# jolars/sgdnet

Measured on AMD Instinct MI355X. Metric: saga_epochs_per_sec, higher is better.
Workload: dtype f64

## Files before the change

sgdnet_amd/csrc/saga_batched.hip:

```cpp
#include <hip/hip_ext.h>
#include <stdlib.h>

#include <mutex>
#include <set>
#include <type_traits>
#include <utility>

#include "device_math.hpp"
#include "r_rng_word.hpp"
#include "r_rng_bodies.hpp"

#ifndef SGDNET_BIN_BLOCK
#define SGDNET_BIN_BLOCK 1024
#endif
#ifndef SGDNET_BIN_W
#define SGDNET_BIN_W 8
#endif
#ifndef SGDNET_RANGE_BLOCK
#define SGDNET_RANGE_BLOCK 512
#endif

namespace sgdnet {

namespace {
// ... 423 lines not shown
    }
    if (y_in_tag && y[i] != 0.0) bits |= 2u;
    if (bits) atomicOr(meta + (i >> 4), bits << (2 * (i & 15)));
  }
}

__global__ __launch_bounds__(256) void m_move_kernel(SagaDev d, int to_record) {
  for (int64_t i = (int64_t)blockIdx.x * 256 + threadIdx.x; i < d.n; i += (int64_t)gridDim.x * 256) {
    double* r = reinterpret_cast<double*>(d.cP + (size_t)i * kCStride + kCMOff);
    if (to_record) *r = d.M[i];
    else d.M[i] = *r;
  }
}

template <class F>
__device__ __forceinline__ void row_tail_compact(const SagaDev& d, uint32_t sid, int nnz, int gl, int E, F f) {
  const char* qb = d.cQ + (size_t)sid * kCStride;
  for (int e = E + 4 + gl; e < nnz; e += kLanes8) {
    if (e < E + kCQ) {
      f((int64_t) reinterpret_cast<const uint16_t*>(qb + 8)[e - E],
        reinterpret_cast<const double*>(qb + 32)[e - E]);
    } else {
      const int64_t q0 = d.ptr[sid];
      f((int64_t)d.idx[q0 + e], d.val[q0 + e]);
    }
  }
}

#ifndef SGDNET_LDS_BLOCK
#define SGDNET_LDS_BLOCK 1024
#endif
constexpr int kLdsBlock = SGDNET_LDS_BLOCK;

constexpr int kTicket = 32;

struct TicketSource {
  int* counter;
  int lo, hi, m;
  int t = 0;
  bool dynamic;
  __device__ __forceinline__ int next() {
    if (!dynamic) {
      const int b = lo + (t++ * (kLdsBlock / 64) + (int)(threadIdx.x >> 6)) * kTicket;
      return b < hi ? b : m;
    }
    int b = 0;
    if ((threadIdx.x & 63) == 0)
      b = __hip_atomic_fetch_add(counter, kTicket, __ATOMIC_RELAXED, __HIP_MEMORY_SCOPE_WORKGROUP);
    b = lo + __builtin_amdgcn_readfirstlane(b);
    return b < hi ? b : m;
  }
};

struct K1Compact {
  typedef double dpair_t __attribute__((ext_vector_type(2)));
  static constexpr int U = 4;
  int E, in_reg, gl, g, q, slot, id_off, v_off;
  bool y_in_meta, is_owner, in_p, half;
  const char* plane;
  char* P;
  const uint32_t* sp;
  const uint32_t* meta;
  int m;
  TicketSource tk;
  int b_cur, b_nxt;
  uint32_t s_cur, s_nxt;

  __device__ __forceinline__ int own_pos(int base) const { return base + U * g + q < m ? base + U * g + q : base; }
  __device__ __forceinline__ uint32_t tagged(uint32_t sid) const {
    const uint32_t mb = (meta[sid >> 4] >> (2 * (sid & 15))) & 3u;
    return sid | ((mb & 1u) ? kLongBit : 0u) | ((mb & 2u) ? kYBit : 0u);
  }
  static __device__ __forceinline__ int static_tickets() { return 2 * (kLdsBlock / 64) * kTicket; }

  __device__ __forceinline__ void init(const SagaDev& d, const uint32_t* sp_, int m_, int blk, int nblk,
                                       int* ticket_counter) {
    E = d.cE;
    in_reg = E + 4;
    y_in_meta = E == 12;
    gl = threadIdx.x & (kLanes8 - 1);
    g = (threadIdx.x & 63) >> 3;
    q = gl >> 1;
    is_owner = (gl & 1) == 0;
    in_p = gl < 6;
    slot = in_p ? gl : gl - 6;
    P = d.cP;
    plane = in_p ? d.cP : d.cQ;
    id_off = in_p ? 8 * E + 4 * slot : 8 + 4 * slot;
    v_off = in_p ? 16 * slot : 32 + 16 * slot;
    half = in_p && slot == 5 && E == 11;
    sp = sp_;
    meta = d.cmeta;
    m = m_;
    const int share = ((m + nblk - 1) / nblk + kTicket - 1) / kTicket * kTicket;
    tk.counter = ticket_counter;
    tk.lo = blk * share;
    tk.hi = tk.lo + share < m ? tk.lo + share : m;
    tk.m = m;
    tk.dynamic = share >= 4 * (kLdsBlock / 64) * kTicket;
    tk.t = 2;
    const int wave = (int)(threadIdx.x >> 6);
    b_cur = tk.lo + wave * kTicket;
    b_nxt = tk.lo + ((kLdsBlock / 64) + wave) * kTicket;
    if (b_cur >= tk.hi) b_cur = m;
    if (b_nxt >= tk.hi) b_nxt = m;
  }
  __device__ __forceinline__ void request_first() {
    s_cur = b_cur < m ? sp[own_pos(b_cur)] : 0u;
    s_nxt = b_nxt < m ? sp[own_pos(b_nxt)] : 0u;
  }
  __device__ __forceinline__ void begin(const SagaDev& d, const uint32_t* sp_, int m_, int blk, int nblk,
                                        int* ticket_counter) {
    init(d, sp_, m_, blk, nblk, ticket_counter);
    request_first();
  }

  __device__ __forceinline__ void tag_first() {
    if (b_cur < m) s_cur = tagged(s_cur);
  }

  __device__ __forceinline__ double run(const SagaDev& d, double b0, const double* wv, double* Dl) {
    double gct = 0.0;
    while (b_cur < m) {
      const bool v_own = b_cur + U * g + q < m;
      uint32_t su[U];
#pragma unroll
      for (int u = 0; u < U; ++u) su[u] = (uint32_t)__shfl((int)s_cur, 2 * u, kLanes8);
      const uint32_t s_this = s_cur & kIdMask;
      double y_own = (s_cur & kYBit) ? 1.0 : 0.0;
      if (!y_in_meta) y_own = *reinterpret_cast<const double*>(P + (size_t)s_this * kCStride + kCYOff);
      int nnz_own = 0;
      if (s_cur & kLongBit) nnz_own = *reinterpret_cast<const int*>(d.cQ + (size_t)s_this * kCStride);
      uint32_t jf[U];
      dpair_t vf[U];
#pragma unroll
      for (int u = 0; u < U; ++u) {
        const bool on = in_p || (su[u] & kLongBit) != 0;
        const char* base = plane + (size_t)(su[u] & kIdMask) * kCStride;
        jf[u] = 0u;
        vf[u] = dpair_t{0.0, 0.0};
        if (on) {
          jf[u] = *reinterpret_cast<const uint32_t*>(base + id_off);
          vf[u] = *reinterpret_cast<const dpair_t*>(base + v_off);
        }
      }
      const int b_nn = b_nxt < m ? tk.next() : m;
      uint32_t s_nn = 0u;
      if (b_nn < m) s_nn = sp[own_pos(b_nn)];
      if (b_nxt < m) s_nxt = tagged(s_nxt);
      if (half) {
#pragma unroll
        for (int u = 0; u < U; ++u) {
          vf[u].y = 0.0;
          jf[u] &= 0xffffu;
        }
      }
      double acc[U];
#pragma unroll
      for (int u = 0; u < U; ++u) acc[u] = vf[u].x * wv[jf[u] & 0xffffu] + vf[u].y * wv[jf[u] >> 16];
      const bool own_tail = v_own && nnz_own > in_reg;
      const bool any_tail = __ballot(own_tail) != 0;
      if (any_tail) {
#pragma unroll
        for (int u = 0; u < U; ++u) {
          const int nz = __shfl(own_tail ? nnz_own : 0, 2 * u, kLanes8);
          if (nz > in_reg) {
            double a = 0.0;
            row_tail_compact(d, su[u] & kIdMask, nz, gl, E, [&](int64_t j, double v) { a += v * wv[j]; });
            acc[u] += a;
          }
        }
      }
      const bool hi4 = (gl & 4) != 0, hi2 = (gl & 2) != 0;
      const double r0 = (hi4 ? acc[2] : acc[0]) + __shfl_xor(hi4 ? acc[0] : acc[2], 4, kLanes8);
      const double r1 = (hi4 ? acc[3] : acc[1]) + __shfl_xor(hi4 ? acc[1] : acc[3], 4, kLanes8);
      double t = (hi2 ? r1 : r0) + __shfl_xor(hi2 ? r0 : r1, 2, kLanes8);
      t += __shfl_xor(t, 1, kLanes8);
      const double lp = t + b0;
      const double g0 = d.family == SGDNET_BINOMIAL ? 1.0 - y_own - 1.0 / (1.0 + exp(lp)) : lp - y_own;
      double gcp = 0.0;
      if (is_owner && v_own) {
        const double old = __hip_atomic_exchange(reinterpret_cast<double*>(P + (size_t)s_this * kCStride + kCMOff), g0,
                                                 __ATOMIC_RELAXED, __HIP_MEMORY_SCOPE_AGENT);
        gcp = g0 - old;
      }
#pragma unroll
      for (int u = 0; u < U; ++u) {
        const double gc = __shfl(gcp, 2 * u, kLanes8);
        if (gc != 0.0) {
          if (vf[u].x != 0.0) scatter_add<true>(Dl + (jf[u] & 0xffffu), vf[u].x * gc);
          if (vf[u].y != 0.0) scatter_add<true>(Dl + (jf[u] >> 16), vf[u].y * gc);
          if (any_tail) {
            const int nz = __shfl(own_tail ? nnz_own : 0, 2 * u, kLanes8);
            if (nz > in_reg)
              row_tail_compact(d, su[u] & kIdMask, nz, gl, E,
                               [&](int64_t j, double v) { scatter_add<true>(Dl + j, v * gc); });
          }
        }
      }
      gct += gcp;
      s_cur = s_nxt;
      s_nxt = s_nn;
      b_cur = b_nxt;
      b_nxt = b_nn;
    }
    return gct;
  }
};

template <int U>
struct K1IdsOnly {
  uint32_t s[U];
  bool valid[U];
  uint32_t s_own;
  bool v_own;
  bool valid_any;
  __device__ __forceinline__ void load(const SagaDev& d, const uint32_t* sp, int i, int hi, int step, int gl,
                                       int safe) {
#pragma unroll
    for (int u = 0; u < U; ++u) {
      const int iu = i + u * step;
      valid[u] = iu < hi;
      s[u] = sp[valid[u] ? iu : safe];
    }
    const int q = U == 4 ? gl >> 2 : gl;
    const int iq = i + q * step;
    v_own = q < U && iq < hi;
    s_own = sp[v_own ? iq : safe];
  }
};

template <int U>
struct K1Draws {
  uint32_t s[U];
  int jf[U], nnz[U];
  double vf[U];
  double gcp;
  bool valid[U];
  uint32_t s_own;
  double y_own;
  bool v_own;
  static __device__ __forceinline__ int draw_of(int gl) { return U == 4 ? gl >> 2 : gl; }

  static __device__ __forceinline__ int owner(int u) { return U == 4 ? 4 * u : u; }
  static __device__ __forceinline__ bool is_owner(int gl) { return U == 4 ? (gl & 3) == 0 : gl < U; }

  __device__ __forceinline__ void load_ids(const SagaDev& d, const uint32_t* sp, int i, int hi, int step, int gl,
                                           int safe) {
#pragma unroll
    for (int u = 0; u < U; ++u) {
      const int iu = i + u * step;
      valid[u] = iu < hi;
      s[u] = sp[valid[u] ? iu : safe];
      if (SGD_ABLATE(d, 16)) s[u] &= 1023u;
    }
    const int q = draw_of(gl);
    const int iq = i + q * step;
    v_own = q < U && iq < hi;
    s_own = sp[v_own ? iq : safe];
    if (SGD_ABLATE(d, 16)) s_own &= 1023u;
  }
// ... 1240 lines not shown
  const int S = d.v_bps, V = d.V;
  if ((int)blockIdx.x >= V * S) {
    if (d.rngdev && lamp->rng_generate) {
      const RngDev* R = d.rngdev;
      const unsigned gen = R->gen;
      uint32_t* lds = reinterpret_cast<uint32_t*>(Dl);
      const int rb = (int)blockIdx.x - V * S, nrb = (int)gridDim.x - V * S;
      mt_state_body(rb, nrb, reinterpret_cast<uint32_t(*)[2][kMtN + 1]>(lds), R->state[gen & 1u], R->ends,
                    R->stream + (int64_t)(gen & 1u) * R->n, R->n, R->seg, R->gens);
      __syncthreads();
      mt_jump_body(rb, nrb, lds, R->state[gen & 1u], R->state[(gen + 1u) & 1u], R->poly, R->gens);
    }
    fused_leave(d, lamp, nb, false);
    return;
  }
  const int v = (int)blockIdx.x % V, wi = (int)blockIdx.x / V;
  const int F = 2 * (int)((p + 2 * S - 1) / (2 * S));
  const int j0 = wi * F;
  const int jn = p - j0 < F ? (p - j0 > 0 ? (int)(p - j0) : 0) : F;
  double* Wl = Dl + p;
  f64x2_t* D2 = reinterpret_cast<f64x2_t*>(Dl);
  f64x2_t* W2 = reinterpret_cast<f64x2_t*>(Wl);
  const int penalty = lamp->penalty;
  __shared__ double sh_par[10];
  if (tid == 0) {
    sh_par[0] = lamp->gamma;
    sh_par[1] = lamp->beta;
    sh_par[2] = lamp->r_full;
    sh_par[3] = lamp->ls_full;
    sh_par[4] = lamp->r_tail;
    sh_par[5] = lamp->ls_tail;
    double tot = 0.0, lo = 0.0;
    for (int u = 0; u < d.V; ++u) {
      tot += d.v_size[u];
      if (u < (int)blockIdx.x % d.V) lo += d.v_size[u];
    }
    sh_par[6] = d.v_size[(int)blockIdx.x % d.V];
    sh_par[7] = lo;
    sh_par[8] = tot;
  }
  const int64_t m_full = lamp->m_full;
  const int64_t sbase = lamp->stream_base;
  const bool raw_words = lamp->stream_raw != 0;
  const int64_t dps = d.v_dps;
  const bool std_x = d.standardize != 0;
  const int64_t L = 2 * p + 2;
  double* vwv = d.vw + (int64_t)v * p;
  double* vGv = d.vG + (int64_t)v * p;
  double* refv = d.vx + (int64_t)v * L;
  double* cwp = d.vx + (int64_t)V * L;
  unsigned* sync = d.vsync;
  const __amdgpu_buffer_rsrc_t rs_slab = fused_rsrc(d.slab, (int64_t)V * S * p * 8);
  const __amdgpu_buffer_rsrc_t rs_w = fused_rsrc(vwv, p * 8);
  uint32_t* const stream_v = const_cast<uint32_t*>(d.stream) + sbase + (int64_t)v * dps;
  constexpr int kC = 8;
  auto conv_range = [&](int m, int& lo, int& hi) {
    const int share = ((m + S - 1) / S + kTicket - 1) / kTicket * kTicket;
    lo = wi * share;
    hi = lo + share < m ? lo + share : m;
  };
  auto conv_load = [&](int64_t t0, int m, uint32_t (&x)[kC]) {
    int lo, hi;
    conv_range(m, lo, hi);
    const uint32_t* q = stream_v + t0;
#pragma unroll
    for (int c = 0; c < kC; ++c) {
      const int i = lo + (int)threadIdx.x + c * kLdsBlock;
      x[c] = i < hi ? q[i] : 0u;
    }
  };
  auto conv_store = [&](int64_t t0, int m, const uint32_t (&x)[kC]) {
    int lo, hi;
    conv_range(m, lo, hi);
    uint32_t* q = stream_v + t0;
    const double n_d = sh_par[6], lo_v = sh_par[7];
#pragma unroll
    for (int c = 0; c < kC; ++c) {
      const int i = lo + (int)threadIdx.x + c * kLdsBlock;
      if (i < hi) q[i] = (uint32_t)lo_v + word_to_draw(x[c], n_d);
    }
    for (int i = lo + (int)threadIdx.x + kC * kLdsBlock; i < hi; i += kLdsBlock)
      q[i] = (uint32_t)lo_v + word_to_draw(q[i], n_d);
  };

#ifdef SGDNET_PHASE_TIMING
  unsigned long long ph_t = 0;
  if (d.dbg && tid == 0) d.dbg[(size_t)blockIdx.x * 16 + 14] = ph_t = phase_stamp();
#define FPH(slot)                                                 \
  do {                                                            \
    if (d.dbg && tid == 0) {                                      \
      const unsigned long long now = phase_stamp();               \
      d.dbg[(size_t)blockIdx.x * 16 + (slot)] += now - ph_t;      \
      d.dbg[(size_t)blockIdx.x * 16 + 15] = ph_t = now;           \
    }                                                             \
  } while (0)
#else
#define FPH(slot) ((void)0)
#endif
  if (tid == 0) {
    const unsigned xcc = __builtin_amdgcn_s_getreg((3 << 11) | 20) & 15u;
    __hip_atomic_fetch_or(sync + (kSyncXcd + v) * kSyncLine, 1u << xcc, __ATOMIC_RELAXED, __HIP_MEMORY_SCOPE_AGENT);
    asm volatile("s_waitcnt vmcnt(0)" ::: "memory");
    __hip_atomic_fetch_add(sync + kSyncStart * kSyncLine, 1u, __ATOMIC_RELAXED, __HIP_MEMORY_SCOPE_AGENT);
    sh_ok = fused_start(sync, lamp, (unsigned)(V * S)) ? 1 : 0;
    if (sh_ok) {
      const unsigned mask = sync_load(sync, kSyncXcd + v);
      sh_ok = (mask & (mask - 1u)) == 0u ? 3 : 1;
    }
  }
  for (int64_t i = tid; i < P2; i += kLdsBlock) D2[i] = f64x2_t{0.0, 0.0};
  __syncthreads();
  bool done = false;
  bool alive = sh_ok != 0;
  unsigned col_base = 0u;
  if (kPeers) {
    int merges = 0;
    for (int r = 0; r < nb; ++r) merges += (r + 1 == nb || (r + 1) % every == 0) ? 1 : 0;
    col_base = sync_load(sync, kSyncSeq) * (unsigned)merges;
  }
  const bool local = (sh_ok & 2) != 0 && d.vs_xcd_local != 0;
  int mi = 0;
  uint32_t s_first = 0u, s_second = 0u;
  if (alive) {
    const int m0 = (int)(dps < m_full ? dps : m_full);
    if (raw_words) {
      uint32_t x0[kC];
      conv_load(0, m0, x0);
      conv_store(0, m0, x0);
      asm volatile("s_waitcnt vmcnt(0)" ::: "memory");
      __syncthreads();
    }
    K1Compact nx;
    nx.begin(d, stream_v, m0, wi, S, &ticket_counter);
    s_first = nx.s_cur;
    s_second = nx.s_nxt;
  }
  for (int r = 0; alive && r < nb; ++r) {
    const int64_t t0 = (int64_t)r * m_full;
    const int m = (int)(dps - t0 < m_full ? dps - t0 : m_full);
    const bool tail = m != m_full;
    const bool last = r + 1 == nb;
    const bool merge_due = last || (r + 1) % every == 0;

    if (tid == 0) ticket_counter = K1Compact::static_tickets();
    K1Compact cg;
    cg.init(d, stream_v + t0, m, wi, S, &ticket_counter);
    cg.s_cur = s_first;
    cg.s_nxt = s_second;
    cg.tag_first();
    int ts = threadIdx.x;
    asm volatile("" : "+v"(ts));
    double cw = 0.0, bv = 0.0;
    if ((ts >> 6) == 0) {
      if (std_x && r > 0)
        for (int k = ts & 63; k < S; k += 64) cw += ld_sc1(cwp + v * kFusedMaxBps + k);
      bv = r == 0 ? d.b[0] : ld_sc1(d.vb + v);
    }
    {
      constexpr int kStage = 8;
      for (int64_t i0 = ts; i0 < P2; i0 += (int64_t)kLdsBlock * kStage) {
        f64x2_t t[kStage];
#pragma unroll
        for (int q = 0; q < kStage; ++q) {
          const int64_t i = i0 + (int64_t)q * kLdsBlock;
          t[q] = f64x2_t{0.0, 0.0};
          if (i < P2) t[q] = r == 0 ? reinterpret_cast<const f64x2_t*>(d.w)[i] : ld2_sc1(rs_w, (uint32_t)(i * 16));
        }
#pragma unroll
        for (int q = 0; q < kStage; ++q) {
          const int64_t i = i0 + (int64_t)q * kLdsBlock;
          if (i < P2) W2[i] = t[q];
        }
      }
    }
    if ((ts >> 6) == 0) {
      cw = wave_sum(cw);
      if ((ts & 63) == 0) sh_val[0] = bv - cw;
    }
    __syncthreads();
    if (r == 0 && std_x) {
      double a = 0.0;
      for (int64_t j = ts; j < p; j += kLdsBlock) a += d.c[j] * Wl[j];
      a = fused_block_sum(a, sh_red);
      if (ts == 0) sh_val[0] -= a;
      __syncthreads();
    }
    const double b0 = sh_val[0];
    FPH(0);

    const double gct = cg.run(d, b0, Wl, Dl);
    __syncthreads();
    FPH(1);
    int tq = threadIdx.x;
    asm volatile("" : "+v"(tq));
    const int lane = tq & 63, wave = tq >> 6;
    const int64_t t0n = t0 + m_full;
    const int mn = (int)(dps - t0n < m_full ? dps - t0n : m_full);
    uint32_t xraw[kC];
    const bool conv_next = !last && raw_words;

    {
      const uint32_t base = (uint32_t)(((int64_t)blockIdx.x * p) * 8);
      for (int64_t i = tq; i < P2; i += kLdsBlock) {
        st2_shard(D2[i], rs_slab, base + (uint32_t)(i * 16), local);
        D2[i] = f64x2_t{0.0, 0.0};
      }
      const double t = wave_sum(gct);
      if (lane == 0) sh_red[wave] = t;
      __syncthreads();
      if (tq == 0) {
        double tot = 0.0;
        for (int wv = 0; wv < kLdsBlock / 64; ++wv) tot += sh_red[wv];
        st_shard(d.vd0 + blockIdx.x, tot, local);
      }
    }
    fused_arrive(sync, kSyncCnt1 + v);
    FPH(2);
    if (conv_next) conv_load(t0n, mn, xraw);
    const bool upd = tq < jn;
    const bool icpt = wi == 0 && tq == jn;
    const bool act = upd || icpt;
    const int64_t j = j0 + tq;
    const int64_t oa = upd ? j : 2 * p, ob = upd ? p + j : 2 * p + 1;
    double* const rep_a = upd ? vGv + j : d.vgb + v;
    double* const rep_b = upd ? vwv + j : d.vb + v;
    const double* const own_a = upd ? d.G + j : d.gb;
    const double* const own_b = upd ? d.w + j : d.b;
    double a_old = 0.0, b_old = 0.0, c_own = 0.0, ra = 0.0, rb = 0.0;
    if (act) {
      a_old = r == 0 ? *own_a : ld_sc1(rep_a);
      b_old = r == 0 ? *own_b : ld_sc1(rep_b);
      if (std_x && upd) c_own = d.c[j];
      if (merge_due) {
        ra = mi == 0 ? *own_a : ld_sc1(refv + oa);
        rb = mi == 0 ? *own_b : ld_sc1(refv + ob);
      }
    }
    if (tq == 0) sh_ok = fused_poll(sync, kSyncCnt1 + v, (unsigned)S * (unsigned)(r + 1), lamp) ? 1 : 0;
    __syncthreads();
    if (!sh_ok) break;
    FPH(3);
    if (conv_next) conv_store(t0n, mn, xraw);

    {
      double gsum = 0.0;
      if (wave == kLdsBlock / 64 - 1)
        for (int k = lane; k < S; k += 64) gsum += ld_sc1(d.vd0 + k * V + v);
      f64x2_t acc[kFusedChunks];
#pragma unroll
      for (int c = 0; c < kFusedChunks; ++c) acc[c] = f64x2_t{0.0, 0.0};
      for (int k = wave; k < S; k += 2 * (kLdsBlock / 64)) {
        const bool two = k + kLdsBlock / 64 < S;
        const uint32_t o0 = (uint32_t)((((int64_t)(k * V + v)) * p + j0) * 8);
        const uint32_t o1 = (uint32_t)((((int64_t)((k + kLdsBlock / 64) * V + v)) * p + j0) * 8);
        f64x2_t a0[kFusedChunks], a1[kFusedChunks];
#pragma unroll
        for (int c = 0; c < kFusedChunks; ++c) {
          const int pi = c * 64 + lane;
          a0[c] = a1[c] = f64x2_t{0.0, 0.0};
          if (2 * pi < jn) {
            a0[c] = ld2_sc1(rs_slab, o0 + (uint32_t)(pi * 16));
            if (two) a1[c] = ld2_sc1(rs_slab, o1 + (uint32_t)(pi * 16));
          }
        }
#pragma unroll
        for (int c = 0; c < kFusedChunks; ++c) {
          acc[c] += a0[c];
          acc[c] += a1[c];
        }
      }
#pragma unroll
      for (int c = 0; c < kFusedChunks; ++c) {
        const int pi = c * 64 + lane;
        if (2 * pi < F) reinterpret_cast<f64x2_t*>(Wl + (int64_t)wave * F)[pi] = acc[c];
      }
      if (wave == kLdsBlock / 64 - 1) {
        gsum = wave_sum(gsum);
        if (lane == 0) sh_val[1] = gsum;
      }
    }
    __syncthreads();
    double a_new = a_old, b_new = b_old;
    {
      const double d0 = sh_val[1];
      const double n_d = sh_par[6], gamma = sh_par[0];
      if (upd) {
        double dj = 0.0;
#pragma unroll
        for (int wv = 0; wv < kLdsBlock / 64; ++wv) dj += Wl[(int64_t)wv * F + tq];
        if (std_x) dj -= c_own * d0;
        const double beta = sh_par[1];
        const double r_m = tail ? sh_par[4] : sh_par[2], ls_m = tail ? sh_par[5] : sh_par[3];
        const double val = r_m * b_old - (gamma * ls_m) * a_old - gamma * dj;
        const double tau = beta * gamma * ls_m;
        b_new = val;
// ... 36 lines not shown
        sh_ok = fused_poll(d.vcol, wi, (unsigned)(NP * V) * (col_base + (unsigned)(mi + 1)), lamp, PR != nullptr, sync) ? 1 : 0;
      __syncthreads();
      if (!sh_ok) break;
      double ma = ra, mb = rb;
      const double tot_all = PR ? PR->tot_size : sh_par[8];
      for (int q = 0; q < NP; ++q) {
        const double* pub0 = (PR ? PR->pub[q] : d.vpub) + (int64_t)((mi & 1) * V) * L;
        double xa[8], xb[8];
#pragma unroll
        for (int u = 0; u < 8; ++u) {
          xa[u] = xb[u] = 0.0;
          if (u < V && act) {
            xa[u] = PR ? ld_sys(pub0 + (int64_t)u * L + oa) : ld_sc1(pub0 + (int64_t)u * L + oa);
            xb[u] = PR ? ld_sys(pub0 + (int64_t)u * L + ob) : ld_sc1(pub0 + (int64_t)u * L + ob);
          }
        }
#pragma unroll
        for (int u = 0; u < 8; ++u) {
          if (u < V) {
            const double wt = (PR ? PR->vsize[q][u] : d.v_size[u]) / tot_all;
            ma += wt * (xa[u] - ra);
            mb += wt * (xb[u] - rb);
          }
        }
      }
      if (act) {
        a_new = ma;
        b_new = mb;
        st_sc1(refv + oa, ma);
        st_sc1(refv + ob, mb);
        if (last && v == 0) {
          *const_cast<double*>(own_a) = ma;
          *const_cast<double*>(own_b) = mb;
        }
      }
      ++mi;
      FPH(5);
    }
    if (act) {
      st_shard(rep_a, a_new, local);
      st_shard(rep_b, b_new, local);
    }
    if (std_x) {
      const double a = fused_block_sum(upd ? c_own * b_new : 0.0, sh_red);
      if (tq == 0) st_shard(cwp + v * kFusedMaxBps + wi, a, local);
    }
    if (last) {
      done = true;
      break;
    }
    fused_arrive(sync, kSyncCnt2 + v);
    FPH(6);
    {
      K1Compact nx;
      nx.begin(d, stream_v + t0n, mn, wi, S, &ticket_counter);
      s_first = nx.s_cur;
      s_second = nx.s_nxt;
    }
    if (tq == 0) sh_ok = fused_poll(sync, kSyncCnt2 + v, (unsigned)S * (unsigned)(r + 1), lamp) ? 1 : 0;
    __syncthreads();
    if (!sh_ok) break;
    FPH(7);
  }

  fused_leave(d, lamp, nb, done);
}

__global__ __launch_bounds__(kBlock) void saga_convergence_kernel(SagaDev d, LamParams* lamp) {
  const int64_t len = (int64_t)d.K * d.p;
  double max_change = 0.0, max_size = 0.0;
  for (int64_t i = (int64_t)blockIdx.x * kBlock + threadIdx.x; i < len; i += (int64_t)gridDim.x * kBlock) {
    const double v = d.w[i];
    max_change = fmax(max_change, fabs(v - d.w_prev[i]));
    max_size = fmax(max_size, fabs(v));
    d.w_prev[i] = v;
  }
  max_change = wave_max(max_change);
  max_size = wave_max(max_size);
  if ((threadIdx.x & 63) == 0) {
    atomic_max_bits(&lamp->max_change_bits, max_change);
    atomic_max_bits(&lamp->max_size_bits, max_size);
  }
}

template <bool kSparse>
__global__ __launch_bounds__(kBlock) void saga_loss_kernel(SagaDev d, LamParams* lamp) {
  extern __shared__ __attribute__((aligned(16))) char smem[];
  double* lps = reinterpret_cast<double*>(smem);
  const int K = d.K;
  const int gl = threadIdx.x & (kGroup - 1);
  const int gib = threadIdx.x / kGroup;
  const int64_t group = ((int64_t)blockIdx.x * kBlock + threadIdx.x) / kGroup;
  const int64_t ngroups = (int64_t)gridDim.x * (kBlock / kGroup);
  double* lp = lps + (size_t)gib * K;
  double* cw = lps + (size_t)(kBlock / kGroup) * K;
  if (kSparse && d.standardize) {
    __shared__ double red[kBlock / 64];
    for (int k = 0; k < K; ++k) {
      double a = 0.0;
      for (int64_t j = threadIdx.x; j < d.p; j += kBlock) a += d.w[k + j * K] * d.c[j];
      a = wave_sum(a);
      if ((threadIdx.x & 63) == 0) red[threadIdx.x >> 6] = a;
      __syncthreads();
      if (threadIdx.x == 0) {
        double t = 0.0;
        for (int wv = 0; wv < kBlock / 64; ++wv) t += red[wv];
        cw[k] = t;
// ... 1031 lines not shown
```

sgdnet_amd/csrc/solver.cpp:

```cpp
#include <math.h>
#include <stdarg.h>
#include <stdlib.h>
#include <stdio.h>
#include <string.h>

#include <algorithm>
#include <string>
#include <chrono>
#include <atomic>
#include <vector>

#include <hip/hip_ext.h>

#include "common.hpp"
#include "setup_device.hpp"

namespace sgdnet {

static thread_local std::string g_last_error;

void set_error(const char* fmt, ...) {
  char buf[1024];
  va_list ap;
  va_start(ap, fmt);
// ... 334 lines not shown
    SGD_HIP_TRY(hipStreamSynchronize(s->st));
    if (s->bin_bufs[1]) (void)hipFree(s->bin_bufs[1]);
    s->bin_bufs[1] = nullptr;
    SGD_HIP_TRY(hipMalloc(&s->bin_bufs[1], sizeof(double) * (size_t)batch * (size_t)d.K));
    s->bin_batch = batch;
    drop_graph(s);
  }
  d.gcb = static_cast<double*>(s->bin_bufs[1]);
  d.KS = d.K;
  return SGDNET_OK;
}

static BatchPlan plan(const sgdnet_solver* s, int64_t batch, int64_t m) {
  return plan_batch(s->d, (int)m, PlanInputs{batch, s->bin_disabled, !s->fused_off && option(kOptFusedEpoch) != 0, s->cus});
}
static bool sharded(const BatchPlan& g) { return g.form == BatchForm::kShards || g.form == BatchForm::kFusedEpoch; }
static bool fused_epochs(const sgdnet_solver* s) { return plan(s, 1, 1).form == BatchForm::kFusedEpoch; }

int set_batch_shape(sgdnet_solver* s, int64_t batch, int64_t draws) {
  if (batch < 1) batch = 1;
  {
    const int rcm = m_to_record(s);
    if (rcm) return rcm;
  }
  const bool shards = sharded(plan(s, batch, batch));
  const int64_t per_launch = shards ? draws / s->d.V : draws;
  if (shards) s->d.v_dps = per_launch;
  if (batch > per_launch) batch = per_launch;
  if (!shards) {
    int rcb = ensure_binned(s, batch);
    if (!rcb) rcb = ensure_dense_tiled(s, batch);
    if (rcb) return rcb;
  }
  const int64_t full = per_launch / batch;
  const int64_t tail = per_launch - full * batch;
  int64_t slab_need = plan(s, batch, batch).slab_doubles;
  if (tail > 0) slab_need = std::max(slab_need, plan(s, batch, tail).slab_doubles);
  if (slab_need > s->slab_cap) {
    SGD_HIP_TRY(hipStreamSynchronize(s->st));
    if (s->d.slab) SGD_HIP_TRY(hipFree(s->d.slab));
    s->d.slab = nullptr;
    SGD_HIP_TRY(hipMalloc(reinterpret_cast<void**>(&s->d.slab), sizeof(double) * (size_t)slab_need));
    s->slab_cap = slab_need;
    drop_graph(s);
  }
  s->lam.m_full = batch;
  s->lam.m_tail = tail;
  batch_factors(s->lam.alpha, s->lam.gamma, batch, &s->lam.r_full, &s->lam.ls_full);
  batch_factors(s->lam.alpha, s->lam.gamma, tail, &s->lam.r_tail, &s->lam.ls_tail);
  s->lam.draws_per_epoch = draws;
  return SGDNET_OK;
}

int prepare_stream_slot(sgdnet_solver* s, int64_t batch, int64_t stream_offset, int64_t draws, int n_epochs) {
  auto& P = s->pipe;
  s->lam.stream_raw = 0;
  s->lam.rng_generate = 0;
  if (!P.open) return SGDNET_OK;
  const bool one_slot = n_epochs == 1 && draws == P.n && (stream_offset == 0 || stream_offset == P.n);
  const int slot = stream_offset == 0 ? 0 : 1;
  const bool fused = one_slot && plan(s, batch, batch).form == BatchForm::kFusedEpoch;
  if (fused && s->d.rngdev && P.pending_gen >= 0 && P.pending_gen == P.used + 1 && slot == (int)(P.used & 1)) {
    s->lam.rng_generate = 1;
    P.pending_gen = -1;
  }
  if (!(P.raw[0] || P.raw[1])) return SGDNET_OK;
  if (fused && P.raw[slot]) {
    s->lam.stream_raw = 1;
    P.raw[slot] = false;
    return SGDNET_OK;
  }
  for (int q = 0; q < 2; ++q) {
    if (!P.raw[q] || (one_slot && q != slot)) continue;
    if (P.pending_gen >= 0 && (int)(P.pending_gen & 1) == q) continue;
    if (!one_slot) SGD_HIP_TRY(hipStreamSynchronize(P.st));
    int rc = launch_rng_convert(s->stream_dev + (int64_t)q * P.n, P.n, (uint32_t)s->d.n, s->st, s->d.V, s->d.v_size,
                                P.run_len);
    if (rc) return rc;
    P.raw[q] = false;
  }
  return SGDNET_OK;
}

int n_batches(int64_t batch, int64_t draws) {
  if (batch < 1) batch = 1;
  if (batch > draws) batch = draws;
  return (int)((draws + batch - 1) / batch);
}

int vs_merge_batches(const sgdnet_solver* s, int64_t batch) {
  const int64_t period = s->vs_period > 0 ? s->vs_period : s->d.n / 32;
  const int64_t b = period / batch;
  return (int)(b < 1 ? 1 : b);
}

int enqueue_epoch_kernels_vs(sgdnet_solver* s, int64_t batch, int64_t draws, std::vector<hipEvent_t>* ev) {
  SagaDev& d = s->d;
  const int64_t dps = draws / d.V;
  if (batch > dps) batch = dps;
  const int nb = n_batches(batch, dps);
  const BatchPlan full = plan(s, batch, batch);
  const int every = vs_merge_batches(s, batch);
  if (full.form == BatchForm::kFusedEpoch) {
    s->d.vs_xcd_local = option(kOptFusedEpoch) == 1 ? 1 : 0;
    if (ev) {
      hipEvent_t e[2];
      for (auto& x : e) SGD_HIP_TRY(hipEventCreate(&x));
      int rcf = launch_vs_epoch(d, full, s->lam_dev, nb, every, s->st, e[0], e[1]);
      if (rcf) return rcf;
      hipEvent_t z[2];
      for (auto& x : z) SGD_HIP_TRY(hipEventCreate(&x));
      SGD_HIP_TRY(hipEventRecord(z[0], s->st));
      SGD_HIP_TRY(hipEventRecord(z[1], s->st));
      ev->push_back(e[0]);
      ev->push_back(e[1]);
      ev->push_back(z[0]);
      ev->push_back(z[1]);
      return SGDNET_OK;
    }
    if (s->time_epochs) {
      hipEvent_t e[2];
      for (auto& x : e) SGD_HIP_TRY(hipEventCreate(&x));
      s->epoch_ev.push_back(e[0]);
      s->epoch_ev.push_back(e[1]);
      return launch_vs_epoch(d, full, s->lam_dev, nb, every, s->st, e[0], e[1]);
    }
    return launch_vs_epoch(d, full, s->lam_dev, nb, every, s->st);
  }
  const BatchPlan tail_plan = plan(s, batch, dps - (int64_t)(nb - 1) * batch);
  int rc = launch_vs_broadcast(d, s->st);
  if (rc) return rc;
  rc = launch_vs_cw(d, s->st);
// ... 130 lines not shown
  return SGDNET_OK;
}

int check_stream(const sgdnet_solver* s, int64_t off, int64_t need) {
  if (!s->stream_dev || off < 0 || off + need > s->stream_len) {
    set_error("sample stream too short: need [%lld, %lld) but %lld entries are resident",
              (long long)off, (long long)(off + need), (long long)s->stream_len);
    return SGDNET_ESTREAM;
  }
  return SGDNET_OK;
}

int read_convergence(sgdnet_solver* s, double tol, int* converged) {
  LamParams back;
  SGD_HIP_TRY(hipMemcpyAsync(&back, s->lam_dev, sizeof(LamParams), hipMemcpyDeviceToHost, s->st));
  SGD_HIP_TRY(hipStreamSynchronize(s->st));
  double max_change, max_size;
  memcpy(&max_change, &back.max_change_bits, 8);
  memcpy(&max_size, &back.max_size_bits, 8);
  const bool all_zero = (max_size == 0.0) && (max_change == 0.0);
  const bool no_change = (max_size != 0.0) && (max_change / max_size <= tol);
  *converged = (all_zero || no_change) ? 1 : 0;
  s->last_change = max_change;
  s->last_size = max_size;
  s->fused_abort_seen = back.fused_abort;
  return SGDNET_OK;
}

int fused_recover(sgdnet_solver* s, int code, int64_t draws, int batches, bool* rerun) {
  *rerun = false;
  if (!code) return SGDNET_OK;
  s->fused_off = true;
  s->fused_abort_seen = 0;
  SGD_HIP_TRY(hipMemsetAsync(reinterpret_cast<char*>(s->lam_dev) + offsetof(LamParams, fused_abort), 0, sizeof(int), s->st));
  SGD_HIP_TRY(hipMemsetAsync(s->d.vsync + vs_fused_sync_sticky_word(), 0, sizeof(unsigned), s->st));
  if (code != 1) {
    set_error("batched mode: a wait inside the fused epoch kernel timed out (internal error; the epoch is void)");
    return SGDNET_EHIP;
  }
  if (s->d.n_peers > 1) {
    set_error("batched mode: the epoch kernel of a linked solver could not become resident on its GPU (shared with other "
              "work?); the ranks' replicas are averaged inside that kernel, so there is no fallback");
    return SGDNET_EHIP;
  }
  if (getenv("SGDNET_TRACE"))
    fprintf(stderr, "[sgdnet]   the fused epoch launch could not become resident (GPU shared?): separate launches from now on\n");
  for (LamParams* q : {&s->lam, &s->lam_dev_mirror}) {
    int64_t sb = q->stream_base - draws;
    if (sb < 0 && q->stream_wrap > 0) sb += q->stream_wrap;
    q->stream_base = sb;
    q->batch_seq -= batches;
  }
  if (s->lam.stream_raw) {
    const int64_t sb = s->lam.stream_base;
    int rc = launch_rng_convert(s->stream_dev + sb, s->pipe.n, (uint32_t)s->d.n, s->st, s->d.V, s->d.v_size, s->pipe.run_len);
    if (rc) return rc;
    s->lam.stream_raw = 0;
  }
  *rerun = true;
  return SGDNET_OK;
}

int device_convergence(sgdnet_solver* s, double tol, int* converged) {
  const size_t off = offsetof(LamParams, max_change_bits);
  SGD_HIP_TRY(hipMemsetAsync(reinterpret_cast<char*>(s->lam_dev) + off, 0, 16, s->st));
  int rc = launch_convergence(s->d, s->lam_dev, s->st);
  if (rc) return rc;
  return read_convergence(s, tol, converged);
}

int device_loss_sum(sgdnet_solver* s, double* out) {
  const size_t off = offsetof(LamParams, loss_acc);
  SGD_HIP_TRY(hipMemsetAsync(reinterpret_cast<char*>(s->lam_dev) + off, 0, 8, s->st));
  int rc = launch_loss(s->d, s->lam_dev, s->sparse, s->st);
  if (rc) return rc;
  SGD_HIP_TRY(hipMemcpyAsync(out, reinterpret_cast<char*>(s->lam_dev) + off, 8, hipMemcpyDeviceToHost,
                             s->st));
  SGD_HIP_TRY(hipStreamSynchronize(s->st));
  return SGDNET_OK;
}

int ensure_ls_table(sgdnet_solver* s, int64_t nit) {
  if (s->LS_dev && s->LS_len == nit + 1 && s->LS_alpha == s->lam.alpha && s->LS_gamma == s->lam.gamma)
    return SGDNET_OK;
  std::vector<double> ls((size_t)(nit + 1 > 2 ? nit + 1 : 2));
  ls[0] = 0.0;
  ls[1] = 1.0;
  double geo = 1.0;
  const double upd = 1.0 - s->lam.alpha * s->lam.gamma;
  for (int64_t i = 2; i < nit + 1; ++i) {
    geo *= upd;
    ls[(size_t)i] = ls[(size_t)i - 1] + geo;
  }
  if (!s->LS_dev || s->LS_len != nit + 1) {
    if (s->LS_dev) {
      SGD_HIP_TRY(hipStreamSynchronize(s->st));
      SGD_HIP_TRY(hipFree(s->LS_dev));
      s->LS_dev = nullptr;
    }
    SGD_HIP_TRY(hipMalloc(reinterpret_cast<void**>(&s->LS_dev), sizeof(double) * ls.size()));
  }
  SGD_HIP_TRY(hipMemcpy(s->LS_dev, ls.data(), sizeof(double) * ls.size(), hipMemcpyHostToDevice));
  s->LS_len = nit + 1;
  s->LS_alpha = s->lam.alpha;
  s->LS_gamma = s->lam.gamma;
  return SGDNET_OK;
}

// ... 452 lines not shown
    set_error("sgdnet_solver_upload_stream: entry %u is not a sample index (n_samples = %lld)", top,
              (long long)s->d.n);
    return SGDNET_EINVAL;
  }
  SGD_HIP_TRY(hipSetDevice(s->device));
  int rc = reserve_stream(s, count);
  if (rc) return rc;
  SGD_HIP_TRY(hipMemcpyAsync(s->stream_dev, host, sizeof(uint32_t) * (size_t)count, hipMemcpyHostToDevice,
                             s->st));
  SGD_HIP_TRY(hipStreamSynchronize(s->st));
  return SGDNET_OK;
}

int sgdnet_solver_rng_open(sgdnet_solver* s, sgdnet_rng* rng, int64_t draws_per_epoch, int generators) {
  if (!s || !rng || draws_per_epoch <= 0) {
    set_error("sgdnet_solver_rng_open: invalid argument");
    return SGDNET_EINVAL;
  }
  int rc = solver_rng_open(s, rng, draws_per_epoch, generators);
  if (rc) return rc;
  return solver_rng_prefetch(s);
}

int sgdnet_solver_rng_layout(sgdnet_solver* s, int64_t draws_per_run) {
  if (!s || draws_per_run < 0) return SGDNET_EINVAL;
  if (s->pipe.open) {
    set_error("sgdnet_solver_rng_layout: set the layout before sgdnet_solver_rng_open");
    return SGDNET_EINVAL;
  }
  s->pipe.run_len = draws_per_run;
  return SGDNET_OK;
}

int sgdnet_solver_rng_next(sgdnet_solver* s, int64_t* stream_offset) {
  if (!s || !stream_offset) return SGDNET_EINVAL;
  int rc = solver_rng_prefetch(s);
  if (rc) return rc;
  return solver_rng_acquire(s, stream_offset);
}

int sgdnet_solver_rng_done(sgdnet_solver* s) { return s ? solver_rng_release(s) : SGDNET_EINVAL; }

int sgdnet_solver_rng_close(sgdnet_solver* s, sgdnet_rng* rng) {
  if (!s || !rng) return SGDNET_EINVAL;
  return solver_rng_close(s, rng);
}

int sgdnet_solver_get_stream(sgdnet_solver* s, uint32_t* host, int64_t offset, int64_t count) {
  if (!s || !host || offset < 0 || count <= 0 || offset + count > s->stream_len) {
    set_error("sgdnet_solver_get_stream: range outside the resident stream");
    return SGDNET_EINVAL;
  }
  SGD_HIP_TRY(hipSetDevice(s->device));
  SGD_HIP_TRY(hipMemcpyAsync(host, s->stream_dev + offset, sizeof(uint32_t) * (size_t)count,
                             hipMemcpyDeviceToHost, s->st));
  SGD_HIP_TRY(hipStreamSynchronize(s->st));
  return SGDNET_OK;
}

int sgdnet_solver_generate_stream(sgdnet_solver* s, sgdnet_rng* rng, int64_t count) {
  if (!s || !rng || count <= 0) {
    set_error("sgdnet_solver_generate_stream: invalid argument");
    return SGDNET_EINVAL;
  }
  SGD_HIP_TRY(hipSetDevice(s->device));
  int rc = reserve_stream(s, count);
  if (rc) return rc;
  if (!s->rng_dev) SGD_HIP_TRY(hipMalloc(reinterpret_cast<void**>(&s->rng_dev), sizeof(sgdnet_rng)));
  static_assert(sizeof(sgdnet_rng) == 625 * sizeof(uint32_t), "sgdnet_rng is mti + 624 words");
  SGD_HIP_TRY(hipMemcpyAsync(s->rng_dev, rng, sizeof(sgdnet_rng), hipMemcpyHostToDevice, s->st));
  rc = launch_rng_fill(s->rng_dev, s->rng_dev, (uint32_t)s->d.n, s->stream_dev, count, s->st, s->d.V, s->d.v_size);
  if (rc) return rc;
  SGD_HIP_TRY(hipMemcpyAsync(rng, s->rng_dev, sizeof(sgdnet_rng), hipMemcpyDeviceToHost, s->st));
  SGD_HIP_TRY(hipStreamSynchronize(s->st));
  return SGDNET_OK;
}

}

bool solver_fused_aborted(const sgdnet_solver* s) { return s && s->fused_abort_seen != 0; }
bool solver_bin_overflowed(const sgdnet_solver* s) { return s && s->bin_overflowed; }

int solver_grow_bins(sgdnet_solver* s) {
  s->bin_overflowed = false;
  if (s->bin_slack < 64.0) {
    s->bin_slack *= 2.0;
    return SGDNET_OK;
  }
  s->bin_disabled = true;
  if (s->d.K > 16) {
    set_error("batched mode: the binned form keeps overflowing and more than 16 classes have no other batched form");
    return SGDNET_EUNSUPPORTED;
  }
  return SGDNET_OK;
}

bool solver_batched_available(sgdnet_solver* s, int64_t batch) {
  if (!s) return false;
  if (s->d.K <= 16) return true;
  if (s->d.K > 64) return false;
  if (!s->sparse) return true;
  if (ensure_binned(s, batch < 1 ? 1 : batch) != SGDNET_OK) return false;
  return s->d.R > 0 && !s->bin_disabled;
}

int solver_reset_state(sgdnet_solver* s, const double* b0) {
// ... 74 lines not shown
  if (generators > 1 && s->d.V > 1 && s->d.vsync) {
    if (!P.dev) SGD_HIP_TRY(hipMalloc(reinterpret_cast<void**>(&P.dev), sizeof(RngDev)));
    RngDev h{};
    h.state[0] = P.state[0];
    h.state[1] = P.state[1];
    h.ends = P.ends;
    h.stream = s->stream_dev;
    h.poly = P.poly_n;
    h.n = n;
    h.seg = seg;
    h.gens = generators;
    h.gen = 0u;
    SGD_HIP_TRY(hipMemcpy(P.dev, &h, sizeof(RngDev), hipMemcpyHostToDevice));
    want = P.dev;
  }
  if (want != s->d.rngdev) {
    s->d.rngdev = want;
    drop_graph(s);
  }
  P.open = true;
  return SGDNET_OK;
}

static int rng_side_generate(sgdnet_solver* s, int64_t g, bool keep_raw) {
  auto& P = s->pipe;
  const int slot = (int)(g & 1);
  SGD_HIP_TRY(hipStreamWaitEvent(P.st, P.freed[slot], 0));
  int rc;
  P.raw[slot] = keep_raw;
  if (P.G > 1) {
    rc = launch_rng_fill(P.state[g & 1], P.ends, (uint32_t)s->d.n, s->stream_dev + (int64_t)slot * P.n, P.n,
                         P.st, s->d.V, s->d.v_size, P.G, P.run_len, keep_raw ? 0 : 1, 0, s->d.cu_reserve);
    if (!rc) rc = launch_rng_jump(P.state[g & 1], P.state[(g + 1) & 1], P.poly_n, P.G, P.st,
                                  std::max(1, s->d.cu_reserve));
  } else {
    rc = launch_rng_fill(P.state[g & 1], P.state[(g + 1) & 1], (uint32_t)s->d.n,
                         s->stream_dev + (int64_t)slot * P.n, P.n, P.st, s->d.V, s->d.v_size, P.G, P.run_len,
                         keep_raw ? 0 : 1);
  }
  if (rc) return rc;
  if (P.dev)
    SGD_HIP_TRY(hipMemsetD32Async(reinterpret_cast<hipDeviceptr_t>(&P.dev->gen), (int)(g + 1), 1, P.st));
  SGD_HIP_TRY(hipEventRecord(P.ready[slot], P.st));
  return SGDNET_OK;
}

int solver_rng_prefetch(sgdnet_solver* s) {
  auto& P = s->pipe;
  if (!P.open || P.gens > P.used + 1) return SGDNET_EINVAL;
  SGD_HIP_TRY(hipSetDevice(s->device));
  const bool keep_raw = P.run_len == 0 && fused_epochs(s);
  if (keep_raw && P.dev && s->d.rngdev && P.G > 1 && P.gens >= 1 && P.pending_gen < 0) {
    P.pending_gen = P.gens;
    P.raw[P.gens & 1] = true;
    ++P.gens;
    return SGDNET_OK;
  }
  int rc = rng_side_generate(s, P.gens, keep_raw);
  if (rc) return rc;
  ++P.gens;
  return SGDNET_OK;
}

int solver_rng_acquire(sgdnet_solver* s, int64_t* offset) {
  auto& P = s->pipe;
  if (!P.open || P.gens <= P.used) return SGDNET_EINVAL;
  const int slot = (int)(P.used & 1);
  if (P.pending_gen == P.used) {
    const int64_t g = P.pending_gen;
    P.pending_gen = -1;
    SGD_HIP_TRY(hipEventRecord(P.freed[slot], s->st));
    int rc = rng_side_generate(s, g, P.raw[slot]);
    if (rc) return rc;
  }
  SGD_HIP_TRY(hipStreamWaitEvent(s->st, P.ready[slot], 0));
  *offset = (int64_t)slot * P.n;
  return SGDNET_OK;
}

int solver_rng_release(sgdnet_solver* s) {
  auto& P = s->pipe;
  SGD_HIP_TRY(hipEventRecord(P.freed[P.used & 1], s->st));
  ++P.used;
  return SGDNET_OK;
}

int solver_rng_close(sgdnet_solver* s, sgdnet_rng* rng) {
  auto& P = s->pipe;
  if (!P.open) return SGDNET_OK;
  SGD_HIP_TRY(hipSetDevice(s->device));
  if (P.pending_gen >= 0) {
    P.raw[P.pending_gen & 1] = false;
    --P.gens;
    P.pending_gen = -1;
  }
  SGD_HIP_TRY(hipStreamSynchronize(P.st));
  SGD_HIP_TRY(hipStreamSynchronize(s->st));
  SGD_HIP_TRY(hipMemcpy(rng, P.state[P.used & 1], sizeof(sgdnet_rng), hipMemcpyDeviceToHost));
  for (int q = 0; q < 2; ++q) {
    if (!P.raw[q]) continue;
    int rcq = launch_rng_convert(s->stream_dev + (int64_t)q * P.n, P.n, (uint32_t)s->d.n, s->st, s->d.V, s->d.v_size, P.run_len);
    if (rcq) return rcq;
    P.raw[q] = false;
  }
  P.open = false;
  if (s->d.rngdev) {
    s->d.rngdev = nullptr;
    drop_graph(s);
  }
  if (s->d.cu_reserve) {
    s->d.cu_reserve = 0;
    if (s->d.V > 1) s->d.v_bps = lds_target_grid(s->d) / s->d.V;
    drop_graph(s);
  }
  return SGDNET_OK;
}

extern "C" {

static int check_bins(sgdnet_solver* s);

int sgdnet_solver_run(sgdnet_solver* s, int mode, int64_t batch, int64_t stream_offset,
                      int64_t draws_per_epoch, unsigned max_epochs, double tol, unsigned* epochs_run,
                      int* converged_out, double* losses) {
  if (!s || draws_per_epoch <= 0 || max_epochs == 0 || !epochs_run || !converged_out) {
    set_error("sgdnet_solver_run: invalid argument");
    return SGDNET_EINVAL;
  }
  if (!s->penalty_set) {
    set_error("sgdnet_solver_run: call sgdnet_solver_set_penalty first");
    return SGDNET_EINVAL;
  }
  SGD_HIP_TRY(hipSetDevice(s->device));
  int rc = check_stream(s, stream_offset, draws_per_epoch);
  if (rc) return rc;
  const size_t wbytes = sizeof(double) * (size_t)s->d.K * (size_t)s->d.p;
  unsigned done = 0;
  int converged = 0;

  if (mode == SGDNET_MODE_EXACT) {
    rc = m_to_array(s);
    if (rc) return rc;
    if (s->sparse) {
      rc = ensure_ls_table(s, draws_per_epoch);
      if (rc) return rc;
    }
    ExactPlan plan;
    rc = plan_exact(s->d, ExactInputs{s->sparse, draws_per_epoch, s->lam.penalty, s->lam.alpha, s->lam.gamma, s->nnz,
                                      option(kOptExactRowRegisters)}, &plan);
    if (rc) return rc;
    while (done < max_epochs && !converged) {
      const int64_t avail = (s->stream_len - stream_offset) / draws_per_epoch;
      if (avail <= 0) {
        set_error("sample stream exhausted after %u epochs", done);
        return SGDNET_ESTREAM;
      }
      unsigned chunk = max_epochs - done;
      if ((int64_t)chunk > avail) chunk = (unsigned)avail;
      if (losses) chunk = 1;
      ExactCtl ctl{};
      ctl.stream_off = stream_offset;
      ctl.nit = draws_per_epoch;
      ctl.max_epochs = chunk;
      ctl.tol = tol;
      ctl.LS = s->LS_dev;
      ctl.use_lds = plan.use_lds;
      ctl.ls_cache = plan.ls_cache;
      ctl.out = s->out_dev;
      rc = launch_exact(s->d, plan, s->lam_dev, ctl, s->st);
      if (rc) return rc;
      int out[2] = {0, 0};
      SGD_HIP_TRY(hipMemcpyAsync(out, s->out_dev, sizeof(out), hipMemcpyDeviceToHost, s->st));
      SGD_HIP_TRY(hipStreamSynchronize(s->st));
      if (out[1] < 0) {
        set_error("exact mode: the sample-order producer of the sparse kernel stalled (internal error)");
        return SGDNET_EHIP;
      }
      if (losses) {
        double sum = 0.0;
        rc = device_loss_sum(s, &sum);
        if (rc) return rc;
        losses[done] = sum / (double)s->d.n;
      }
#ifdef SGDNET_PHASE_TIMING
      if (plan.form == ExactForm::kDenseSmall2 && s->d.dbg && out[0] > 0) {
        unsigned long long c[5];
        SGD_HIP_TRY(hipMemcpy(c, s->d.dbg + 24, sizeof(c), hipMemcpyDeviceToHost));
        (void)hipMemset(s->d.dbg + 24, 0, sizeof(c));
        const double its = (double)out[0] * (double)draws_per_epoch;
        fprintf(stderr, "[sgdnet] small dense kernel with feeder, consumer cycles per draw: slot+history %.0f, dot %.0f, gradient+store %.0f, "
                        "intercept %.0f, step+penalty+average %.0f\n", c[0] / its, c[1] / its, c[2] / its, c[3] / its, c[4] / its);
      }
      if (plan.form == ExactForm::kSparseK1m && s->d.dbg && out[0] > 0) {
        (void)hipDeviceSynchronize();
// ... 804 lines not shown
```

Baseline: 1216.

## Convert raw RNG words to sample indices on the fly inside fused epoch kernel

The fused epoch kernel no longer rewrites the raw RNG word stream into sample indices in place with separate load/store passes between batches. Instead, each sample id is converted when it is consumed in the compact K1 loop, via a templated struct that applies word_to_draw when the stream is raw. Host code now leaves slots marked raw and converts them lazily (before host copies, exact mode, or close) through new helper functions. This removes in-kernel global stores and a barrier, at the cost of redoing the conversion arithmetic on every read and more complex raw-state bookkeeping.

```diff
diff --git a/sgdnet_amd/csrc/saga_batched.hip b/sgdnet_amd/csrc/saga_batched.hip
--- a/sgdnet_amd/csrc/saga_batched.hip
+++ b/sgdnet_amd/csrc/saga_batched.hip
@@ -499,7 +499,8 @@
   }
 };
 
-struct K1Compact {
+template <bool kRawStream>
+struct K1CompactT {
   typedef double dpair_t __attribute__((ext_vector_type(2)));
   static constexpr int U = 4;
   int E, in_reg, gl, g, q, slot, id_off, v_off;
@@ -512,6 +513,13 @@
   TicketSource tk;
   int b_cur, b_nxt;
   uint32_t s_cur, s_nxt;
+  bool raw = false;
+  const double* par = nullptr;
+
+  __device__ __forceinline__ uint32_t sample_id(uint32_t x) const {
+    if (kRawStream && raw) x = (uint32_t)par[1] + word_to_draw(x, par[0]);
+    return x;
+  }
 
   __device__ __forceinline__ int own_pos(int base) const { return base + U * g + q < m ? base + U * g + q : base; }
   __device__ __forceinline__ uint32_t tagged(uint32_t sid) const {
@@ -563,7 +571,7 @@
   }
 
   __device__ __forceinline__ void tag_first() {
-    if (b_cur < m) s_cur = tagged(s_cur);
+    if (b_cur < m) s_cur = tagged(sample_id(s_cur));
   }
 
   __device__ __forceinline__ double run(const SagaDev& d, double b0, const double* wv, double* Dl) {
@@ -594,7 +602,7 @@
       const int b_nn = b_nxt < m ? tk.next() : m;
       uint32_t s_nn = 0u;
       if (b_nn < m) s_nn = sp[own_pos(b_nn)];
-      if (b_nxt < m) s_nxt = tagged(s_nxt);
+      if (b_nxt < m) s_nxt = tagged(sample_id(s_nxt));
       if (half) {
 #pragma unroll
         for (int u = 0; u < U; ++u) {
@@ -654,6 +662,7 @@
     return gct;
   }
 };
+typedef K1CompactT<false> K1Compact;
 
 template <int U>
 struct K1IdsOnly {
@@ -2000,36 +2009,9 @@
   unsigned* sync = d.vsync;
   const __amdgpu_buffer_rsrc_t rs_slab = fused_rsrc(d.slab, (int64_t)V * S * p * 8);
   const __amdgpu_buffer_rsrc_t rs_w = fused_rsrc(vwv, p * 8);
-  uint32_t* const stream_v = const_cast<uint32_t*>(d.stream) + sbase + (int64_t)v * dps;
-  constexpr int kC = 8;
-  auto conv_range = [&](int m, int& lo, int& hi) {
-    const int share = ((m + S - 1) / S + kTicket - 1) / kTicket * kTicket;
-    lo = wi * share;
-    hi = lo + share < m ? lo + share : m;
-  };
-  auto conv_load = [&](int64_t t0, int m, uint32_t (&x)[kC]) {
-    int lo, hi;
-    conv_range(m, lo, hi);
-    const uint32_t* q = stream_v + t0;
-#pragma unroll
-    for (int c = 0; c < kC; ++c) {
-      const int i = lo + (int)threadIdx.x + c * kLdsBlock;
-      x[c] = i < hi ? q[i] : 0u;
-    }
-  };
-  auto conv_store = [&](int64_t t0, int m, const uint32_t (&x)[kC]) {
-    int lo, hi;
-    conv_range(m, lo, hi);
-    uint32_t* q = stream_v + t0;
-    const double n_d = sh_par[6], lo_v = sh_par[7];
-#pragma unroll
-    for (int c = 0; c < kC; ++c) {
-      const int i = lo + (int)threadIdx.x + c * kLdsBlock;
-      if (i < hi) q[i] = (uint32_t)lo_v + word_to_draw(x[c], n_d);
-    }
-    for (int i = lo + (int)threadIdx.x + kC * kLdsBlock; i < hi; i += kLdsBlock)
-      q[i] = (uint32_t)lo_v + word_to_draw(q[i], n_d);
-  };
+  const uint32_t* const stream_v = d.stream + sbase + (int64_t)v * dps;
+  typedef K1CompactT<true> K1Epoch;
+  const double* const draw_par = sh_par + 6;
 
 #ifdef SGDNET_PHASE_TIMING
   unsigned long long ph_t = 0;
@@ -2071,14 +2053,7 @@
   uint32_t s_first = 0u, s_second = 0u;
   if (alive) {
     const int m0 = (int)(dps < m_full ? dps : m_full);
-    if (raw_words) {
-      uint32_t x0[kC];
-      conv_load(0, m0, x0);
-      conv_store(0, m0, x0);
-      asm volatile("s_waitcnt vmcnt(0)" ::: "memory");
-      __syncthreads();
-    }
-    K1Compact nx;
+    K1Epoch nx;
     nx.begin(d, stream_v, m0, wi, S, &ticket_counter);
     s_first = nx.s_cur;
     s_second = nx.s_nxt;
@@ -2090,9 +2065,11 @@
     const bool last = r + 1 == nb;
     const bool merge_due = last || (r + 1) % every == 0;
 
-    if (tid == 0) ticket_counter = K1Compact::static_tickets();
-    K1Compact cg;
+    if (tid == 0) ticket_counter = K1Epoch::static_tickets();
+    K1Epoch cg;
     cg.init(d, stream_v + t0, m, wi, S, &ticket_counter);
+    cg.raw = raw_words;
+    cg.par = draw_par;
     cg.s_cur = s_first;
     cg.s_nxt = s_second;
     cg.tag_first();
@@ -2144,8 +2121,6 @@
     const int lane = tq & 63, wave = tq >> 6;
     const int64_t t0n = t0 + m_full;
     const int mn = (int)(dps - t0n < m_full ? dps - t0n : m_full);
-    uint32_t xraw[kC];
-    const bool conv_next = !last && raw_words;
 
     {
       const uint32_t base = (uint32_t)(((int64_t)blockIdx.x * p) * 8);
@@ -2164,7 +2139,6 @@
     }
     fused_arrive(sync, kSyncCnt1 + v);
     FPH(2);
-    if (conv_next) conv_load(t0n, mn, xraw);
     const bool upd = tq < jn;
     const bool icpt = wi == 0 && tq == jn;
     const bool act = upd || icpt;
@@ -2188,7 +2162,6 @@
     __syncthreads();
     if (!sh_ok) break;
     FPH(3);
-    if (conv_next) conv_store(t0n, mn, xraw);
 
     {
       double gsum = 0.0;
@@ -2331,7 +2304,7 @@
     fused_arrive(sync, kSyncCnt2 + v);
     FPH(6);
     {
-      K1Compact nx;
+      K1Epoch nx;
       nx.begin(d, stream_v + t0n, mn, wi, S, &ticket_counter);
       s_first = nx.s_cur;
       s_second = nx.s_nxt;
diff --git a/sgdnet_amd/csrc/solver.cpp b/sgdnet_amd/csrc/solver.cpp
--- a/sgdnet_amd/csrc/solver.cpp
+++ b/sgdnet_amd/csrc/solver.cpp
@@ -410,6 +410,28 @@
   return SGDNET_OK;
 }
 
+static int slot_to_draws(sgdnet_solver* s, int q) {
+  auto& P = s->pipe;
+  if (!P.raw[q]) return SGDNET_OK;
+  SGD_HIP_TRY(hipStreamWaitEvent(s->st, P.ready[q], 0));
+  int rc = launch_rng_convert(s->stream_dev + (int64_t)q * P.n, P.n, (uint32_t)s->d.n, s->st, s->d.V, s->d.v_size,
+                              P.run_len);
+  if (rc) return rc;
+  P.raw[q] = false;
+  return SGDNET_OK;
+}
+
+static int stream_to_draws(sgdnet_solver* s, int64_t offset, int64_t count) {
+  auto& P = s->pipe;
+  if (!P.open || !(P.raw[0] || P.raw[1])) return SGDNET_OK;
+  for (int q = 0; q < 2; ++q) {
+    if (offset >= (int64_t)(q + 1) * P.n || offset + count <= (int64_t)q * P.n) continue;
+    int rc = slot_to_draws(s, q);
+    if (rc) return rc;
+  }
+  return SGDNET_OK;
+}
+
 int prepare_stream_slot(sgdnet_solver* s, int64_t batch, int64_t stream_offset, int64_t draws, int n_epochs) {
   auto& P = s->pipe;
   s->lam.stream_raw = 0;
@@ -420,22 +442,19 @@
   const bool fused = one_slot && plan(s, batch, batch).form == BatchForm::kFusedEpoch;
   if (fused && s->d.rngdev && P.pending_gen >= 0 && P.pending_gen == P.used + 1 && slot == (int)(P.used & 1)) {
     s->lam.rng_generate = 1;
+    P.raw[P.pending_gen & 1] = true;
     P.pending_gen = -1;
   }
   if (!(P.raw[0] || P.raw[1])) return SGDNET_OK;
   if (fused && P.raw[slot]) {
     s->lam.stream_raw = 1;
-    P.raw[slot] = false;
     return SGDNET_OK;
   }
   for (int q = 0; q < 2; ++q) {
     if (!P.raw[q] || (one_slot && q != slot)) continue;
-    if (P.pending_gen >= 0 && (int)(P.pending_gen & 1) == q) continue;
     if (!one_slot) SGD_HIP_TRY(hipStreamSynchronize(P.st));
-    int rc = launch_rng_convert(s->stream_dev + (int64_t)q * P.n, P.n, (uint32_t)s->d.n, s->st, s->d.V, s->d.v_size,
-                                P.run_len);
+    int rc = slot_to_draws(s, q);
     if (rc) return rc;
-    P.raw[q] = false;
   }
   return SGDNET_OK;
 }
@@ -672,8 +691,7 @@
     q->batch_seq -= batches;
   }
   if (s->lam.stream_raw) {
-    const int64_t sb = s->lam.stream_base;
-    int rc = launch_rng_convert(s->stream_dev + sb, s->pipe.n, (uint32_t)s->d.n, s->st, s->d.V, s->d.v_size, s->pipe.run_len);
+    int rc = stream_to_draws(s, s->lam.stream_base, s->pipe.n);
     if (rc) return rc;
     s->lam.stream_raw = 0;
   }
@@ -1232,6 +1250,8 @@
     return SGDNET_EINVAL;
   }
   SGD_HIP_TRY(hipSetDevice(s->device));
+  int rc = stream_to_draws(s, offset, count);
+  if (rc) return rc;
   SGD_HIP_TRY(hipMemcpyAsync(host, s->stream_dev + offset, sizeof(uint32_t) * (size_t)count,
                              hipMemcpyDeviceToHost, s->st));
   SGD_HIP_TRY(hipStreamSynchronize(s->st));
@@ -1412,7 +1432,6 @@
   const bool keep_raw = P.run_len == 0 && fused_epochs(s);
   if (keep_raw && P.dev && s->d.rngdev && P.G > 1 && P.gens >= 1 && P.pending_gen < 0) {
     P.pending_gen = P.gens;
-    P.raw[P.gens & 1] = true;
     ++P.gens;
     return SGDNET_OK;
   }
@@ -1430,7 +1449,7 @@
     const int64_t g = P.pending_gen;
     P.pending_gen = -1;
     SGD_HIP_TRY(hipEventRecord(P.freed[slot], s->st));
-    int rc = rng_side_generate(s, g, P.raw[slot]);
+    int rc = rng_side_generate(s, g, true);
     if (rc) return rc;
   }
   SGD_HIP_TRY(hipStreamWaitEvent(s->st, P.ready[slot], 0));
@@ -1450,7 +1469,6 @@
   if (!P.open) return SGDNET_OK;
   SGD_HIP_TRY(hipSetDevice(s->device));
   if (P.pending_gen >= 0) {
-    P.raw[P.pending_gen & 1] = false;
     --P.gens;
     P.pending_gen = -1;
   }
@@ -1458,10 +1476,8 @@
   SGD_HIP_TRY(hipStreamSynchronize(s->st));
   SGD_HIP_TRY(hipMemcpy(rng, P.state[P.used & 1], sizeof(sgdnet_rng), hipMemcpyDeviceToHost));
   for (int q = 0; q < 2; ++q) {
-    if (!P.raw[q]) continue;
-    int rcq = launch_rng_convert(s->stream_dev + (int64_t)q * P.n, P.n, (uint32_t)s->d.n, s->st, s->d.V, s->d.v_size, P.run_len);
+    int rcq = slot_to_draws(s, q);
     if (rcq) return rcq;
-    P.raw[q] = false;
   }
   P.open = false;
   if (s->d.rngdev) {
@@ -1500,6 +1516,8 @@
 
   if (mode == SGDNET_MODE_EXACT) {
     rc = m_to_array(s);
+    if (rc) return rc;
+    rc = stream_to_draws(s, stream_offset, s->stream_len - stream_offset);
     if (rc) return rc;
     if (s->sparse) {
       rc = ensure_ls_table(s, draws_per_epoch);
```

New measurement: 1305 (median of 6 runs). 7.3% higher.
